# Lqm26/BMCNet-ESR

Hardware: AMD Instinct MI355X
Metric: LR-voxel-frames/sec x4 SR train step, NFS-shaped 180x240 (BASELINE configs[1] / [2]), f32 (higher is better)
Workload: dtype f32; 1 GPU; BMCNet(scale=4, n_c=128, n_b=5) x4 SR train step, NFS-shaped 180x240 (BASELINE configs[1] / [2]) -> 720x960, bs=4/GPU, arithmetic fp32 (native fp32 MFMA; 3x3 convolutions through Winograd F(4x4,3x3) / F(2x2,3x3) transforms in fp32), SEQL=9 SEQN=2 (8 windows BPTT), event scatter + fwd + MSE + bwd + Adam(amsgrad); global_batch=4, parallelism=dp1, rccl_ranks=1, rccl_initialised_before_headline_run=False

## Files before the change

### bmcnet-esr_amd/csrc/conv1p.hip

```cpp
#include "bmc_common.h"
#include "conv_k.h"
#include "dma_ring.h"
#include "tile_walk.h"
#include <stdlib.h>

namespace {

constexpr int CK = BMC_CK;
constexpr int PX = 64;
constexpr int CHF = PX * CK;

template <int NCH, int DEPTH>
__global__ __launch_bounds__(512, (NCH == 8 && DEPTH == 1) ? 4 : 2) void conv1p_kernel(const ConvK a) {
    constexpr int SLOT = NCH * CHF;
    constexpr int NS = DEPTH + 1;
    __shared__ __attribute__((aligned(16))) float lds[NS * SLOT + BMC_MAX_SRC * 8];
    SrcDev* const tab = reinterpret_cast<SrcDev*>(lds + NS * SLOT);
    const unsigned x_lds = lds_addr(lds);
    const int tid = threadIdx.x, lane = tid & 63, wave = __builtin_amdgcn_readfirstlane(tid >> 6);
    const int li = lane & 15, lk = lane >> 4;
    BMC_LOAD_SRC_TABLE(tab, a, tid);
    __syncthreads();

    const int HW = a.H * a.W;
    const int tpi = (HW + PX - 1) / PX;
    const TileWalk tw = tile_walk(a.ntiles);
    const int t_first = tw.first, t_hi = tw.hi, t_stride = tw.stride;
    if (t_first >= t_hi) return;
    using TileIt = Tile2;
    auto decode = [&](int t) { return tile_decode(t, a.ntn, tpi); };
    const TileIt stp = decode(t_stride);
    auto advance = [&](TileIt it) { return tile_advance(it, stp, a.ntn, tpi); };

    const int lpx = (wave & 3) * 16 + (lane >> 2);
    const unsigned lq = (unsigned)(((lane & 3) ^ swz(lane >> 2)) * 4);
    const char* xbase[NCH / 2];
    unsigned xstride[NCH / 2];
    int xl_b = -1;
    auto loader_image = [&](int b) {
        int s_idx = 0, c_in = (wave >> 2) * CK;
#pragma unroll
        for (int j = 0; j < NCH / 2; ++j) {
            while (c_in >= tab[s_idx].nch) { c_in -= tab[s_idx].nch; ++s_idx; }
            const SrcDev S = tab[s_idx];
            xbase[j] = reinterpret_cast<const char*>(src_batch_ptr(S, b) + c_in);
            xstride[j] = (unsigned)S.pix_stride * 4u;
            c_in += 2 * CK;
        }
        xl_b = b;
    };
    auto issue_x_part = [&](const TileIt& it, int slot, int j0, int j1) __attribute__((always_inline)) {
        if (it.b != xl_b) loader_image(it.b);
        int p = it.pt * PX + lpx;
        p = p < HW ? p : HW - 1;
#pragma unroll
        for (int j = j0; j < j1; ++j)
            dma16(xbase[j], (unsigned)p * xstride[j] + lq * 4u,
                  x_lds + (unsigned)((slot * SLOT + ((wave >> 2) + 2 * j) * CHF + (wave & 3) * 256) * 4));
    };
    auto issue_x = [&](const TileIt& it, int slot) { issue_x_part(it, slot, 0, NCH / 2); };

    f32x4 wreg[NCH];
    f32x4 bq = {0.f, 0.f, 0.f, 0.f};
    int w_grp = -1, w_nt = -1;
    const int wq = (lk ^ swz(li)) * 4;
    auto load_w = [&](int grp, int nt) {
        const float* const wb = static_cast<const float*>(a.w) + (long long)grp * a.w_group_stride +
                                ((long long)nt * 128 + 16 * wave + li) * CK + 4 * lk;
        auto ld8 = [](const float* p, long long st, f32x4 (&v)[NCH], int c0) __attribute__((always_inline)) {
            asm volatile("global_load_dwordx4 %0, %8, off\n\tglobal_load_dwordx4 %1, %9, off\n\tglobal_load_dwordx4 %2, %10, off\n\t"
                         "global_load_dwordx4 %3, %11, off\n\tglobal_load_dwordx4 %4, %12, off\n\tglobal_load_dwordx4 %5, %13, off\n\t"
                         "global_load_dwordx4 %6, %14, off\n\tglobal_load_dwordx4 %7, %15, off\n\ts_waitcnt vmcnt(0)"
                         : "=&v"(v[c0]), "=&v"(v[c0 + 1]), "=&v"(v[c0 + 2]), "=&v"(v[c0 + 3]), "=&v"(v[c0 + 4]), "=&v"(v[c0 + 5]),
                           "=&v"(v[c0 + 6]), "=&v"(v[c0 + 7])
                         : "v"(p), "v"(p + st), "v"(p + 2 * st), "v"(p + 3 * st), "v"(p + 4 * st), "v"(p + 5 * st), "v"(p + 6 * st),
                           "v"(p + 7 * st)
                         : "memory");
        };
        const long long wst = (long long)a.Coutpad * CK;
#pragma unroll
        for (int c0 = 0; c0 < NCH; c0 += 8) ld8(wb + c0 * wst, wst, wreg, c0);
        const int co = nt * 128 + 16 * wave + 4 * lk;
        bq = f32x4{0.f, 0.f, 0.f, 0.f};
        if (a.bias && co < a.Cout)
            asm volatile("global_load_dwordx4 %0, %1, off\n\ts_waitcnt vmcnt(0)" : "=v"(bq) : "v"(a.bias + (long long)grp * a.bias_group_stride + co) : "memory");
        w_grp = grp; w_nt = nt;
    };

    const int xoff = li * CK + wq;
    auto read_x = [&](const float* xb, int c, f32x4 (&xf)[4]) __attribute__((always_inline)) {
#pragma unroll
        for (int pb = 0; pb < 4; ++pb) xf[pb] = *reinterpret_cast<const f32x4*>(xb + c * CHF + pb * 16 * CK + xoff);
    };

    int tile = t_first;
    TileIt it = decode(tile);
    TileIt itl = it;
    int tl = t_first, nl = 0;
#pragma unroll
    for (int d = 0; d < DEPTH; ++d) {
        if (tl < t_hi) { issue_x(itl, nl % NS); itl = advance(itl); tl += t_stride; ++nl; }
    }
    dma_wait<0>();
    ring_publish();
    int n = 0;
    int ep_b = -1, grp = 0;
    float* outb = nullptr;
    const float* resb = nullptr;
    const float* maskb = nullptr;
    for (; tile < t_hi; tile += t_stride, ++n) {
        const bool more = tl < t_hi;
        if (it.b != ep_b) {
            ep_b = it.b;
            grp = a.batch_per_group >= a.B ? 0 : it.b / a.batch_per_group;
            outb = a.out + (long long)it.b * a.out_batch_stride;
            resb = a.residual.ptr ? src_batch_ptr(a.residual, it.b) : nullptr;
            maskb = a.mask.ptr ? src_batch_ptr(a.mask, it.b) : nullptr;
        }
        if (grp != w_grp || it.nt != w_nt) load_w(grp, it.nt);

        const int co = it.nt * 128 + 16 * wave + 4 * lk;
        const bool cok = co < a.Cout;
        int pix[4];
        bool ok[4];
#pragma unroll
        for (int pb = 0; pb < 4; ++pb) {
            pix[pb] = it.pt * PX + pb * 16 + li;
            ok[pb] = pix[pb] < HW && cok;
        }
        constexpr bool EPF = NCH == 16;
        f32x4 rv[4], mv[4], ov[4];
        auto ep_load = [&](const float* base, int stride, float fill, f32x4 (&v)[4]) __attribute__((always_inline)) {
#pragma unroll
            for (int pb = 0; pb < 4; ++pb) {
                v[pb] = f32x4{fill, fill, fill, fill};
                if (ok[pb]) v[pb] = ldg16(base + (long long)pix[pb] * stride + co);
            }
        };
        auto ep_request = [&](const float* base, int stride, f32x4 (&v)[4]) __attribute__((always_inline)) {
#pragma unroll
            for (int pb = 0; pb < 4; ++pb) {
                const float* const q = base + (long long)(pix[pb] < HW ? pix[pb] : HW - 1) * stride + (cok ? co : 0);
                asm volatile("global_load_dwordx4 %0, %1, off" : "=v"(v[pb]) : "v"(q) : "memory");
            }
        };
        if (EPF) {
            if (resb) ep_request(resb, a.residual.pix_stride, rv);
            if (maskb) ep_request(maskb, a.mask.pix_stride, mv);
            if (a.accumulate) ep_request(outb, a.out_pix_stride, ov);
        }

        const float* const xb = lds + (n % NS) * SLOT;
        f32x4 acc[4];
#pragma unroll
        for (int pb = 0; pb < 4; ++pb) acc[pb] = bq;
        f32x4 xfA[4], xfB[4];
        read_x(xb, 0, xfA);
#pragma unroll
        for (int c = 0; c < NCH; c += 2) {
            read_x(xb, c + 1, xfB);
#pragma unroll
            for (int j = 0; j < 4; ++j)
#pragma unroll
                for (int pb = 0; pb < 4; ++pb) acc[pb] = __builtin_amdgcn_mfma_f32_16x16x4f32(wreg[c][j], xfA[pb][j], acc[pb], 0, 0, 0);
            if (c + 2 < NCH) read_x(xb, c + 2, xfA);
            if (more && c < NCH / 2) {
                constexpr int PER = (NCH / 2) / (NCH / 4);
                issue_x_part(itl, nl % NS, (c / 2) * PER, (c / 2 + 1) * PER);
                if (c == NCH / 2 - 2) { itl = advance(itl); tl += t_stride; ++nl; }
            }
#pragma unroll
            for (int j = 0; j < 4; ++j)
#pragma unroll
                for (int pb = 0; pb < 4; ++pb) acc[pb] = __builtin_amdgcn_mfma_f32_16x16x4f32(wreg[c + 1][j], xfB[pb][j], acc[pb], 0, 0, 0);
        }

        if (EPF && (resb || maskb || a.accumulate)) {
            if (more) asm volatile("s_waitcnt vmcnt(%0)" :: "n"(NCH / 2) : "memory");
            else asm volatile("s_waitcnt vmcnt(0)" ::: "memory");
#pragma unroll
            for (int pb = 0; pb < 4; ++pb) asm volatile("" : "+v"(rv[pb]), "+v"(mv[pb]), "+v"(ov[pb]));
        }
        if (resb) {
            if (!EPF) ep_load(resb, a.residual.pix_stride, 0.f, rv);
#pragma unroll
            for (int pb = 0; pb < 4; ++pb) acc[pb] += rv[pb];
        }
        if (a.relu) {
#pragma unroll
            for (int pb = 0; pb < 4; ++pb)
#pragma unroll
                for (int k = 0; k < 4; ++k) acc[pb][k] = fmaxf(acc[pb][k], 0.f);
        }
        if (maskb) {
            if (!EPF) ep_load(maskb, a.mask.pix_stride, 1.f, mv);
#pragma unroll
            for (int pb = 0; pb < 4; ++pb)
#pragma unroll
                for (int k = 0; k < 4; ++k) acc[pb][k] = mv[pb][k] > 0.f ? acc[pb][k] : 0.f;
        }
        if (a.accumulate) {
            if (!EPF) ep_load(outb, a.out_pix_stride, 0.f, ov);
#pragma unroll
            for (int pb = 0; pb < 4; ++pb) acc[pb] += ov[pb];
        }
#pragma unroll
        for (int pb = 0; pb < 4; ++pb)
            if (ok[pb]) stg16(outb + (long long)pix[pb] * a.out_pix_stride + co, acc[pb]);
        if (DEPTH > 1 && more) dma_wait<4 + (DEPTH - 1) * (NCH / 2)>(); else dma_wait<4>();
        ring_publish();
        it = advance(it);
    }
}

}

int bmc_conv1p_launch(ConvK k, int cus, hipStream_t st) {
    static const bool off = getenv("BMC_CONV1P") && atoi(getenv("BMC_CONV1P")) == 0;
    if (off || k.Coutpad % 128 != 0 || (k.nchunks != 8 && k.nchunks != 16)) return 0;
    const long long hw = (long long)k.H * k.W;
    k.ntn = k.Coutpad / 128;
    const long long ntiles = (long long)k.B * ((hw + PX - 1) / PX) * k.ntn;
    if (ntiles >= (1ll << 31) || hw * 1024 >= (1ll << 31)) return 0;
    for (int i = 0; i < k.nsrc; ++i)
        if (hw * k.src[i].pix_stride * 4 >= (1ll << 32)) return 0;
    k.ntiles = (int)ntiles;
    const int per_cu = k.nchunks == 8 ? 2 : 1;
    const long long max_blocks = (long long)per_cu * cus;
    dim3 grid((unsigned)(ntiles < max_blocks ? ntiles : max_blocks)), block(512);
    if (k.nchunks == 8) hipLaunchKernelGGL((conv1p_kernel<8, 1>), grid, block, 0, st, k);
    else hipLaunchKernelGGL((conv1p_kernel<16, 1>), grid, block, 0, st, k);
    return 1;
}
```

Before: 48.15 LR-voxel-frames/s.

## Add half-width 4-wave conv1p variant with 32-pixel tiles for K=256

Adds a 256-thread variant of the 1x1 conv kernel for 16-chunk inputs. It uses 32-pixel tiles, and each wave covers two 16-channel output blocks, so weight registers are reused across more MFMAs and LDS per block is halved. Two blocks can then run per CU. Per-lane source pointers are broadcast with readlane to save registers. Weight loads now use an SGPR base plus a VGPR offset, and the tile loop is restructured so weights reload only when the group or n-tile changes. The epilogue reuses register buffers, which may serialize the residual, mask and accumulate loads. The new path is chosen when there are enough tiles, or through BMC_CONV1P_HALF.

```diff
diff --git a/bmcnet-esr_amd/csrc/conv1p.hip b/bmcnet-esr_amd/csrc/conv1p.hip
--- a/bmcnet-esr_amd/csrc/conv1p.hip
+++ b/bmcnet-esr_amd/csrc/conv1p.hip
@@ -7,11 +7,13 @@
 namespace {
 
 constexpr int CK = BMC_CK;
-constexpr int PX = 64;
-constexpr int CHF = PX * CK;
-
-template <int NCH, int DEPTH>
-__global__ __launch_bounds__(512, (NCH == 8 && DEPTH == 1) ? 4 : 2) void conv1p_kernel(const ConvK a) {
+
+template <int NCH, int DEPTH, int NW>
+__global__ __launch_bounds__(64 * NW, (NCH == 8 && DEPTH == 1) ? 4 : 2) void conv1p_kernel(const ConvK a) {
+    static_assert(NW == 8 || (NW == 4 && NCH == 16), "half form: K = 256 only");
+    constexpr int PX = 8 * NW;
+    constexpr int PB = PX / 16, CB = 4 / PB;
+    constexpr int CHF = PX * CK;
     constexpr int SLOT = NCH * CHF;
     constexpr int NS = DEPTH + 1;
     __shared__ __attribute__((aligned(16))) float lds[NS * SLOT + BMC_MAX_SRC * 8];
@@ -32,15 +34,17 @@
     const TileIt stp = decode(t_stride);
     auto advance = [&](TileIt it) { return tile_advance(it, stp, a.ntn, tpi); };
 
-    const int lpx = (wave & 3) * 16 + (lane >> 2);
+    const int lpg = wave % PB, lc0 = wave / PB;
+    const int lpx = lpg * 16 + (lane >> 2);
     const unsigned lq = (unsigned)(((lane & 3) ^ swz(lane >> 2)) * 4);
-    const char* xbase[NCH / 2];
-    unsigned xstride[NCH / 2];
+    constexpr bool LANE_STATE = NW == 4;
+    const char* xbase[LANE_STATE ? 1 : NCH / 2];
+    unsigned xstride[LANE_STATE ? 1 : NCH / 2];
     int xl_b = -1;
     auto loader_image = [&](int b) {
-        int s_idx = 0, c_in = (wave >> 2) * CK;
-#pragma unroll
-        for (int j = 0; j < NCH / 2; ++j) {
+        int s_idx = 0, c_in = (lc0 + (LANE_STATE && lane < NCH / 2 ? 2 * lane : 0)) * CK;
+#pragma unroll
+        for (int j = 0; j < (LANE_STATE ? 1 : NCH / 2); ++j) {
             while (c_in >= tab[s_idx].nch) { c_in -= tab[s_idx].nch; ++s_idx; }
             const SrcDev S = tab[s_idx];
             xbase[j] = reinterpret_cast<const char*>(src_batch_ptr(S, b) + c_in);
@@ -50,47 +54,64 @@
         xl_b = b;
     };
     auto issue_x_part = [&](const TileIt& it, int slot, int j0, int j1) __attribute__((always_inline)) {
-        if (it.b != xl_b) loader_image(it.b);
         int p = it.pt * PX + lpx;
         p = p < HW ? p : HW - 1;
 #pragma unroll
-        for (int j = j0; j < j1; ++j)
-            dma16(xbase[j], (unsigned)p * xstride[j] + lq * 4u,
-                  x_lds + (unsigned)((slot * SLOT + ((wave >> 2) + 2 * j) * CHF + (wave & 3) * 256) * 4));
-    };
-    auto issue_x = [&](const TileIt& it, int slot) { issue_x_part(it, slot, 0, NCH / 2); };
-
-    f32x4 wreg[NCH];
-    f32x4 bq = {0.f, 0.f, 0.f, 0.f};
+        for (int j = j0; j < j1; ++j) {
+            const unsigned dst = x_lds + (unsigned)((slot * SLOT + (lc0 + 2 * j) * CHF + lpg * 256) * 4);
+            if constexpr (LANE_STATE) {
+                const unsigned long long pv = reinterpret_cast<unsigned long long>(xbase[0]);
+                const unsigned lo = __builtin_amdgcn_readlane((unsigned)pv, j), hi = __builtin_amdgcn_readlane((unsigned)(pv >> 32), j);
+                const unsigned stride = __builtin_amdgcn_readlane(xstride[0], j);
+                dma16_sgpr(reinterpret_cast<const void*>(((unsigned long long)hi << 32) | lo), (unsigned)p * stride + lq * 4u,
+                           __builtin_amdgcn_readfirstlane(dst));
+            } else {
+                dma16(xbase[j], (unsigned)p * xstride[j] + lq * 4u, dst);
+            }
+        }
+    };
+    auto issue_x = [&](const TileIt& it, int slot) {
+        if (it.b != xl_b) loader_image(it.b);
+        issue_x_part(it, slot, 0, NCH / 2);
+    };
+
+    f32x4 wreg[CB][NCH];
+    f32x4 bq[CB];
     int w_grp = -1, w_nt = -1;
     const int wq = (lk ^ swz(li)) * 4;
     auto load_w = [&](int grp, int nt) {
-        const float* const wb = static_cast<const float*>(a.w) + (long long)grp * a.w_group_stride +
-                                ((long long)nt * 128 + 16 * wave + li) * CK + 4 * lk;
-        auto ld8 = [](const float* p, long long st, f32x4 (&v)[NCH], int c0) __attribute__((always_inline)) {
-            asm volatile("global_load_dwordx4 %0, %8, off\n\tglobal_load_dwordx4 %1, %9, off\n\tglobal_load_dwordx4 %2, %10, off\n\t"
-                         "global_load_dwordx4 %3, %11, off\n\tglobal_load_dwordx4 %4, %12, off\n\tglobal_load_dwordx4 %5, %13, off\n\t"
-                         "global_load_dwordx4 %6, %14, off\n\tglobal_load_dwordx4 %7, %15, off\n\ts_waitcnt vmcnt(0)"
+        auto ld8 = [](const float* sbase, unsigned& voff, unsigned step, f32x4 (&v)[NCH], int c0) __attribute__((always_inline)) {
+            asm volatile("s_nop 4\n\t"
+                         "global_load_dwordx4 %0, %8, %9\n\tv_add_u32 %8, %10, %8\n\tglobal_load_dwordx4 %1, %8, %9\n\tv_add_u32 %8, %10, %8\n\t"
+                         "global_load_dwordx4 %2, %8, %9\n\tv_add_u32 %8, %10, %8\n\tglobal_load_dwordx4 %3, %8, %9\n\tv_add_u32 %8, %10, %8\n\t"
+                         "global_load_dwordx4 %4, %8, %9\n\tv_add_u32 %8, %10, %8\n\tglobal_load_dwordx4 %5, %8, %9\n\tv_add_u32 %8, %10, %8\n\t"
+                         "global_load_dwordx4 %6, %8, %9\n\tv_add_u32 %8, %10, %8\n\tglobal_load_dwordx4 %7, %8, %9\n\tv_add_u32 %8, %10, %8\n\t"
+                         "s_waitcnt vmcnt(0)"
                          : "=&v"(v[c0]), "=&v"(v[c0 + 1]), "=&v"(v[c0 + 2]), "=&v"(v[c0 + 3]), "=&v"(v[c0 + 4]), "=&v"(v[c0 + 5]),
-                           "=&v"(v[c0 + 6]), "=&v"(v[c0 + 7])
-                         : "v"(p), "v"(p + st), "v"(p + 2 * st), "v"(p + 3 * st), "v"(p + 4 * st), "v"(p + 5 * st), "v"(p + 6 * st),
-                           "v"(p + 7 * st)
+                           "=&v"(v[c0 + 6]), "=&v"(v[c0 + 7]), "+v"(voff)
+                         : "s"(sbase), "s"(step)
                          : "memory");
         };
-        const long long wst = (long long)a.Coutpad * CK;
-#pragma unroll
-        for (int c0 = 0; c0 < NCH; c0 += 8) ld8(wb + c0 * wst, wst, wreg, c0);
-        const int co = nt * 128 + 16 * wave + 4 * lk;
-        bq = f32x4{0.f, 0.f, 0.f, 0.f};
-        if (a.bias && co < a.Cout)
-            asm volatile("global_load_dwordx4 %0, %1, off\n\ts_waitcnt vmcnt(0)" : "=v"(bq) : "v"(a.bias + (long long)grp * a.bias_group_stride + co) : "memory");
+        const unsigned wstep = (unsigned)a.Coutpad * CK * 4u;
+#pragma unroll
+        for (int cb = 0; cb < CB; ++cb) {
+            const float* const wb = static_cast<const float*>(a.w) + (long long)grp * a.w_group_stride +
+                                    ((long long)nt * 128 + 16 * (CB * wave + cb)) * CK;
+            unsigned voff = (unsigned)(li * CK + 4 * lk) * 4u;
+#pragma unroll
+            for (int c0 = 0; c0 < NCH; c0 += 8) ld8(wb, voff, wstep, wreg[cb], c0);
+            const int co = nt * 128 + 16 * (CB * wave + cb) + 4 * lk;
+            bq[cb] = f32x4{0.f, 0.f, 0.f, 0.f};
+            if (a.bias && co < a.Cout)
+                asm volatile("global_load_dwordx4 %0, %1, off\n\ts_waitcnt vmcnt(0)" : "=v"(bq[cb]) : "v"(a.bias + (long long)grp * a.bias_group_stride + co) : "memory");
+        }
         w_grp = grp; w_nt = nt;
     };
 
     const int xoff = li * CK + wq;
-    auto read_x = [&](const float* xb, int c, f32x4 (&xf)[4]) __attribute__((always_inline)) {
-#pragma unroll
-        for (int pb = 0; pb < 4; ++pb) xf[pb] = *reinterpret_cast<const f32x4*>(xb + c * CHF + pb * 16 * CK + xoff);
+    auto read_x = [&](const float* xb, int c, f32x4 (&xf)[PB]) __attribute__((always_inline)) {
+#pragma unroll
+        for (int pb = 0; pb < PB; ++pb) xf[pb] = *reinterpret_cast<const f32x4*>(xb + c * CHF + pb * 16 * CK + xoff);
     };
 
     int tile = t_first;
@@ -108,8 +129,7 @@
     float* outb = nullptr;
     const float* resb = nullptr;
     const float* maskb = nullptr;
-    for (; tile < t_hi; tile += t_stride, ++n) {
-        const bool more = tl < t_hi;
+    auto ep_image = [&]() {
         if (it.b != ep_b) {
             ep_b = it.b;
             grp = a.batch_per_group >= a.B ? 0 : it.b / a.batch_per_group;
@@ -117,44 +137,59 @@
             resb = a.residual.ptr ? src_batch_ptr(a.residual, it.b) : nullptr;
             maskb = a.mask.ptr ? src_batch_ptr(a.mask, it.b) : nullptr;
         }
-        if (grp != w_grp || it.nt != w_nt) load_w(grp, it.nt);
-
-        const int co = it.nt * 128 + 16 * wave + 4 * lk;
-        const bool cok = co < a.Cout;
-        int pix[4];
-        bool ok[4];
-#pragma unroll
-        for (int pb = 0; pb < 4; ++pb) {
-            pix[pb] = it.pt * PX + pb * 16 + li;
-            ok[pb] = pix[pb] < HW && cok;
+    };
+    while (tile < t_hi) {
+      ep_image();
+      load_w(grp, it.nt);
+      do {
+        const bool more = tl < t_hi;
+
+        int co[4], pix[4];
+        bool cok[4], ok[4];
+#pragma unroll
+        for (int t = 0; t < 4; ++t) {
+            co[t] = it.nt * 128 + 16 * (CB * wave + t / PB) + 4 * lk;
+            cok[t] = co[t] < a.Cout;
+            pix[t] = it.pt * PX + (t % PB) * 16 + li;
+            ok[t] = pix[t] < HW && cok[t];
         }
         constexpr bool EPF = NCH == 16;
+        constexpr bool EP1 = NW == 4;
         f32x4 rv[4], mv[4], ov[4];
         auto ep_load = [&](const float* base, int stride, float fill, f32x4 (&v)[4]) __attribute__((always_inline)) {
 #pragma unroll
-            for (int pb = 0; pb < 4; ++pb) {
-                v[pb] = f32x4{fill, fill, fill, fill};
-                if (ok[pb]) v[pb] = ldg16(base + (long long)pix[pb] * stride + co);
+            for (int t = 0; t < 4; ++t) {
+                v[t] = f32x4{fill, fill, fill, fill};
+                if (ok[t]) v[t] = ldg16(base + (long long)pix[t] * stride + co[t]);
             }
         };
         auto ep_request = [&](const float* base, int stride, f32x4 (&v)[4]) __attribute__((always_inline)) {
 #pragma unroll
-            for (int pb = 0; pb < 4; ++pb) {
-                const float* const q = base + (long long)(pix[pb] < HW ? pix[pb] : HW - 1) * stride + (cok ? co : 0);
-                asm volatile("global_load_dwordx4 %0, %1, off" : "=v"(v[pb]) : "v"(q) : "memory");
-            }
-        };
+            for (int t = 0; t < 4; ++t) {
+                const float* const q = base + (long long)(pix[t] < HW ? pix[t] : HW - 1) * stride + (cok[t] ? co[t] : 0);
+                asm volatile("global_load_dwordx4 %0, %1, off" : "=v"(v[t]) : "v"(q) : "memory");
+            }
+        };
+        auto ep_fetch = [&](const float* base, int stride, f32x4 (&v)[4]) __attribute__((always_inline)) {
+            ep_request(base, stride, v);
+            asm volatile("s_waitcnt vmcnt(0)" ::: "memory");
+#pragma unroll
+            for (int t = 0; t < 4; ++t) asm volatile("" : "+v"(v[t]));
+        };
+        const bool mask_ahead = !EP1 || !resb, acc_ahead = !EP1 || (!resb && !maskb);
         if (EPF) {
             if (resb) ep_request(resb, a.residual.pix_stride, rv);
-            if (maskb) ep_request(maskb, a.mask.pix_stride, mv);
-            if (a.accumulate) ep_request(outb, a.out_pix_stride, ov);
-        }
+            if (maskb && mask_ahead) ep_request(maskb, a.mask.pix_stride, EP1 ? rv : mv);
+            if (a.accumulate && acc_ahead) ep_request(outb, a.out_pix_stride, EP1 ? rv : ov);
+        }
+
+        if (more && itl.b != xl_b) loader_image(itl.b);
 
         const float* const xb = lds + (n % NS) * SLOT;
         f32x4 acc[4];
 #pragma unroll
-        for (int pb = 0; pb < 4; ++pb) acc[pb] = bq;
-        f32x4 xfA[4], xfB[4];
+        for (int t = 0; t < 4; ++t) acc[t] = bq[t / PB];
+        f32x4 xfA[PB], xfB[PB];
         read_x(xb, 0, xfA);
 #pragma unroll
         for (int c = 0; c < NCH; c += 2) {
@@ -162,7 +197,7 @@
 #pragma unroll
             for (int j = 0; j < 4; ++j)
 #pragma unroll
-                for (int pb = 0; pb < 4; ++pb) acc[pb] = __builtin_amdgcn_mfma_f32_16x16x4f32(wreg[c][j], xfA[pb][j], acc[pb], 0, 0, 0);
+                for (int t = 0; t < 4; ++t) acc[t] = __builtin_amdgcn_mfma_f32_16x16x4f32(wreg[t / PB][c][j], xfA[t % PB][j], acc[t], 0, 0, 0);
             if (c + 2 < NCH) read_x(xb, c + 2, xfA);
             if (more && c < NCH / 2) {
                 constexpr int PER = (NCH / 2) / (NCH / 4);
@@ -172,44 +207,58 @@
 #pragma unroll
             for (int j = 0; j < 4; ++j)
 #pragma unroll
-                for (int pb = 0; pb < 4; ++pb) acc[pb] = __builtin_amdgcn_mfma_f32_16x16x4f32(wreg[c + 1][j], xfB[pb][j], acc[pb], 0, 0, 0);
+                for (int t = 0; t < 4; ++t) acc[t] = __builtin_amdgcn_mfma_f32_16x16x4f32(wreg[t / PB][c + 1][j], xfB[t % PB][j], acc[t], 0, 0, 0);
         }
 
         if (EPF && (resb || maskb || a.accumulate)) {
             if (more) asm volatile("s_waitcnt vmcnt(%0)" :: "n"(NCH / 2) : "memory");
             else asm volatile("s_waitcnt vmcnt(0)" ::: "memory");
 #pragma unroll
-            for (int pb = 0; pb < 4; ++pb) asm volatile("" : "+v"(rv[pb]), "+v"(mv[pb]), "+v"(ov[pb]));
-        }
+            for (int t = 0; t < 4; ++t) {
+                asm volatile("" : "+v"(rv[t]));
+                if (!EP1) asm volatile("" : "+v"(mv[t]), "+v"(ov[t]));
+            }
+        }
+        auto add = [&](const f32x4 (&v)[4]) __attribute__((always_inline)) {
+#pragma unroll
+            for (int t = 0; t < 4; ++t) acc[t] += v[t];
+        };
+        auto keep_where_positive = [&](const f32x4 (&v)[4]) __attribute__((always_inline)) {
+#pragma unroll
+            for (int t = 0; t < 4; ++t)
+#pragma unroll
+                for (int k = 0; k < 4; ++k) acc[t][k] = v[t][k] > 0.f ? acc[t][k] : 0.f;
+        };
         if (resb) {
             if (!EPF) ep_load(resb, a.residual.pix_stride, 0.f, rv);
-#pragma unroll
-            for (int pb = 0; pb < 4; ++pb) acc[pb] += rv[pb];
+            add(rv);
         }
         if (a.relu) {
 #pragma unroll
-            for (int pb = 0; pb < 4; ++pb)
-#pragma unroll
-                for (int k = 0; k < 4; ++k) acc[pb][k] = fmaxf(acc[pb][k], 0.f);
+            for (int t = 0; t < 4; ++t)
+#pragma unroll
+                for (int k = 0; k < 4; ++k) acc[t][k] = fmaxf(acc[t][k], 0.f);
         }
         if (maskb) {
             if (!EPF) ep_load(maskb, a.mask.pix_stride, 1.f, mv);
-#pragma unroll
-            for (int pb = 0; pb < 4; ++pb)
-#pragma unroll
-                for (int k = 0; k < 4; ++k) acc[pb][k] = mv[pb][k] > 0.f ? acc[pb][k] : 0.f;
+            if (!mask_ahead) ep_fetch(maskb, a.mask.pix_stride, mv);
+            if (EP1 && mask_ahead) keep_where_positive(rv); else keep_where_positive(mv);
         }
         if (a.accumulate) {
             if (!EPF) ep_load(outb, a.out_pix_stride, 0.f, ov);
-#pragma unroll
-            for (int pb = 0; pb < 4; ++pb) acc[pb] += ov[pb];
-        }
-#pragma unroll
-        for (int pb = 0; pb < 4; ++pb)
-            if (ok[pb]) stg16(outb + (long long)pix[pb] * a.out_pix_stride + co, acc[pb]);
+            if (!acc_ahead) ep_fetch(outb, a.out_pix_stride, mv);
+            if (!EP1) add(ov); else if (acc_ahead) add(rv); else add(mv);
+        }
+#pragma unroll
+        for (int t = 0; t < 4; ++t)
+            if (ok[t]) stg16(outb + (long long)pix[t] * a.out_pix_stride + co[t], acc[t]);
         if (DEPTH > 1 && more) dma_wait<4 + (DEPTH - 1) * (NCH / 2)>(); else dma_wait<4>();
         ring_publish();
         it = advance(it);
+        tile += t_stride;
+        ++n;
+        if (tile < t_hi) ep_image();
+      } while (tile < t_hi && grp == w_grp && it.nt == w_nt);
     }
 }
 
@@ -217,18 +266,23 @@
 
 int bmc_conv1p_launch(ConvK k, int cus, hipStream_t st) {
     static const bool off = getenv("BMC_CONV1P") && atoi(getenv("BMC_CONV1P")) == 0;
-    if (off || k.Coutpad % 128 != 0 || (k.nchunks != 8 && k.nchunks != 16)) return 0;
+    if (off || k.Coutpad % 128 != 0 || k.Coutpad >= (1 << 22) || (k.nchunks != 8 && k.nchunks != 16)) return 0;
     const long long hw = (long long)k.H * k.W;
     k.ntn = k.Coutpad / 128;
-    const long long ntiles = (long long)k.B * ((hw + PX - 1) / PX) * k.ntn;
+    const long long tiles32 = (long long)k.B * ((hw + 31) / 32) * k.ntn;
+    const char* const e = getenv("BMC_CONV1P_HALF");
+    const bool half = k.nchunks == 16 && (e && *e ? atoi(e) != 0 : tiles32 >= 2ll * cus);
+    const int px = half ? 32 : 64;
+    const long long ntiles = (long long)k.B * ((hw + px - 1) / px) * k.ntn;
     if (ntiles >= (1ll << 31) || hw * 1024 >= (1ll << 31)) return 0;
     for (int i = 0; i < k.nsrc; ++i)
         if (hw * k.src[i].pix_stride * 4 >= (1ll << 32)) return 0;
     k.ntiles = (int)ntiles;
-    const int per_cu = k.nchunks == 8 ? 2 : 1;
+    const int per_cu = (k.nchunks == 8 || half) ? 2 : 1;
     const long long max_blocks = (long long)per_cu * cus;
-    dim3 grid((unsigned)(ntiles < max_blocks ? ntiles : max_blocks)), block(512);
-    if (k.nchunks == 8) hipLaunchKernelGGL((conv1p_kernel<8, 1>), grid, block, 0, st, k);
-    else hipLaunchKernelGGL((conv1p_kernel<16, 1>), grid, block, 0, st, k);
+    dim3 grid((unsigned)(ntiles < max_blocks ? ntiles : max_blocks)), block(half ? 256 : 512);
+    if (k.nchunks == 8) hipLaunchKernelGGL((conv1p_kernel<8, 1, 8>), grid, block, 0, st, k);
+    else if (half) hipLaunchKernelGGL((conv1p_kernel<16, 1, 4>), grid, block, 0, st, k);
+    else hipLaunchKernelGGL((conv1p_kernel<16, 1, 8>), grid, block, 0, st, k);
     return 1;
 }
```

Result: no change. 48.58 LR-voxel-frames/s (median of 6 runs) (+0.9%).
